# BrooksLabUCSC/splicedice

Measured on AMD Instinct MI355X. Metric: PS-matrix entries/sec (junctions x samples), higher is better.
Workload: dtype int32 counts -> f32 PS; 1 GPU; quant 2000000 junctions x 500 samples per GPU (north_star target size), cluster+PS; junctions_per_gpu=2000000, samples=500, counts=one seeded block of 200000 rows repeated down the matrix, parallelism=junction shards x1, one rank per GPU

## Files before the change

### splicedice_amd/csrc/cluster_fast.hip

```cpp
#include "common.h"

#ifndef SDICE_CLUSTER_ABLATE
#define SDICE_CLUSTER_ABLATE 0
#endif
#define SD_ABL(a, bit) (SDICE_CLUSTER_ABLATE && ((a).ablate & (bit)))

int sd_cluster_legacy(sdice_ctx* ctx, int64_t n, const int32_t* d_chrom, const int32_t* d_left, const int32_t* d_right,
                      const int8_t* d_strand, int32_t* d_row_of, int64_t* d_row_ptr, int64_t* nnz_out);

namespace {

constexpr int SPB = 8;
constexpr int BUCKET_MEAN = 2048;
constexpr int MAX_BUCKETS = 4096;
constexpr int SLOT_FACTOR = 8;
constexpr int64_t FAST_MAX_N = (int64_t)MAX_BUCKETS * BUCKET_MEAN;

enum : unsigned long long { ST_INVALID = 1, ST_SLOT_OVERFLOW = 2, ST_DUP = 4, ST_COL_OVERFLOW = 8, ST_LOOKBACK = 16 };
constexpr int SB_FLAGS = 0, SB_NNZ = 2, SB_MAXLEN = 32, SB_REACH = 64, SB_WORDS = 96;
constexpr int SB_STICKY = SB_WORDS, SB_ALLOC_WORDS = SB_WORDS + 8;
constexpr int SB_SLOTS = 32;

struct FastArgs {
    const int32_t* chrom; const int32_t* left; const int32_t* right; const int8_t* strand;
    int64_t n;
    int B;
    int S;
    int64_t slot_cap;
    int lds_cap;
    unsigned long long* sb;
    uint32_t* rank;
    uint32_t* col_done;
    uint64_t* spl;
    uint32_t* cursor;
    uint4* slots;
    uint32_t* rowC; uint32_t* rowL; uint32_t* rowR2;
    uint32_t* bmax64;
    unsigned long long* tile_state;
    int32_t* row_of; int64_t* row_ptr; int32_t* col; int64_t col_cap;
    uint32_t* blkneed;
    int spb;
    int sample_sort;
    int ablate;
};

__device__ __forceinline__ bool key_less(uint32_t ac, uint32_t al, uint32_t ar, uint32_t bc, uint32_t bl, uint32_t br) {
    return ac < bc || (ac == bc && (al < bl || (al == bl && ar < br)));
}
__device__ __forceinline__ bool elem_less(const uint4& a, const uint4& b) { return key_less(a.x, a.y, a.z, b.x, b.y, b.z); }

__device__ __forceinline__ int64_t sample_pos(int64_t i, int64_t n, int64_t S) {
    const int64_t stride = n / S;
    const uint64_t h = ((uint64_t)i * 0x9E3779B97F4A7C15ull) >> 33;
    return i * stride + (int64_t)(h % (uint64_t)stride);
}

__device__ __forceinline__ uint64_t sample_key(const FastArgs& a, int64_t i) {
    const int64_t p = sample_pos(i, a.n, a.S);
    return ((uint64_t)(uint32_t)a.chrom[p] << 32) | (uint64_t)(uint32_t)a.left[p];
}

__device__ __forceinline__ void count_less96(unsigned& c, uint64_t ka, uint32_t ia, uint64_t kb, uint32_t ib) {
    unsigned t;
    asm("v_sub_co_u32 %0, vcc, %2, %3\n\t"
        "v_subb_co_u32 %0, vcc, %4, %5, vcc\n\t"
        "v_subb_co_u32 %0, vcc, %6, %7, vcc\n\t"
        "v_addc_co_u32 %1, vcc, 0, %1, vcc"
        : "=&v"(t), "+v"(c)
        : "v"(ia), "v"(ib), "v"((unsigned)ka), "v"((unsigned)kb), "v"((unsigned)(ka >> 32)), "v"((unsigned)(kb >> 32))
        : "vcc");
}

__global__ void __launch_bounds__(256) sample_rank_kernel(FastArgs a) {
    __shared__ __align__(16) uint64_t jk[256];
    __shared__ unsigned last;
    const int t = threadIdx.x;
    if (blockIdx.x == 0 && blockIdx.y == 0 && t < SB_WORDS) a.sb[t] = 0ull;
    const int64_t i = (int64_t)blockIdx.x * 256 + t, j = (int64_t)blockIdx.y * 256 + t;
    jk[t] = j < a.S ? sample_key(a, j) : ~0ull;
    const uint64_t ik = i < a.S ? sample_key(a, i) : 0ull;
    __syncthreads();
    const int64_t j0 = (int64_t)blockIdx.y * 256;
    const int64_t split64 = i - j0;
    const uint32_t split = split64 < 0 ? 0u : split64 > 256 ? 256u : (uint32_t)split64;
    uint32_t cnt = 0;
#pragma unroll 8
    for (int q = 0; q < (SD_ABL(a, 8) ? 0 : 256); q += 2) {
        const ulonglong2 k2 = *reinterpret_cast<const ulonglong2*>(&jk[q]);
        count_less96(cnt, k2.x, (uint32_t)q, ik, split);
        count_less96(cnt, k2.y, (uint32_t)q + 1u, ik, split);
    }
    if (i < a.S && cnt) atomicAdd(&a.rank[i], cnt);
    asm volatile("s_waitcnt vmcnt(0)" ::: "memory");
    __syncthreads();
    if (t == 0) last = atomicAdd(&a.col_done[blockIdx.x], 1u) == gridDim.y - 1 ? 1u : 0u;
    __syncthreads();
    if (last && i < a.S) {
        const uint32_t rk = atomicAdd(&a.rank[i], 0u);
        if (rk != 0 && rk % (uint32_t)a.spb == 0) a.spl[rk / (uint32_t)a.spb - 1] = ik;
    }
}

constexpr int SC_KPT = 4;
template <int T>
__global__ void __launch_bounds__(T) bucket_scatter_kernel(FastArgs a) {
    extern __shared__ uint64_t sm64[];
    const int B = a.B;
    uint64_t* spl = sm64;
    uint32_t* cnt = reinterpret_cast<uint32_t*>(sm64 + B);
    uint32_t* base = cnt + B;
    __shared__ uint32_t wmax[T / 64];
    __shared__ uint32_t s_bad, s_over;
    const int t = threadIdx.x;
    if (t == 0) { s_bad = 0; s_over = 0; }
    for (int b = t; b < B; b += T) { spl[b] = b < B - 1 ? a.spl[b] : ~0ull; cnt[b] = 0; }
    __syncthreads();
    const int64_t tile0 = (int64_t)blockIdx.x * T * SC_KPT;
    uint32_t kc[SC_KPT], kl[SC_KPT], kr[SC_KPT], bk[SC_KPT], lr[SC_KPT];
    uint32_t maxlen = 0, bad = 0;
#pragma unroll
    for (int q = 0; q < SC_KPT; ++q) {
        const int64_t i = tile0 + q * T + t;
        bk[q] = 0xffffffffu;
        kc[q] = kl[q] = kr[q] = lr[q] = 0;
        if (i < a.n) {
            const int32_t c = a.chrom[i], l = a.left[i], r = a.right[i];
            const int st = a.strand[i];
            if (l < 0 || r < l || c < 0 || (st != 0 && st != 1)) bad = 1;
            else maxlen = max(maxlen, (uint32_t)(r - l));
            kc[q] = (uint32_t)c; kl[q] = (uint32_t)l; kr[q] = ((uint32_t)r << 1) | (uint32_t)(st & 1);
        }
    }
#pragma unroll
    for (int q = 0; q < SC_KPT; ++q) {
        if (tile0 + q * T + t < a.n) {
            const uint64_t k = ((uint64_t)kc[q] << 32) | kl[q];
            int lo = 0, hi = B - 1;
            while (lo < hi) {
                const int mid = (lo + hi) >> 1;
                if (spl[mid] <= k) lo = mid + 1; else hi = mid;
            }
            bk[q] = (uint32_t)lo;
            lr[q] = atomicAdd(&cnt[lo], 1u);
        }
    }
#pragma unroll
    for (int o = 32; o > 0; o >>= 1) maxlen = max(maxlen, (uint32_t)__shfl_xor((int)maxlen, o));
    if ((t & 63) == 0) wmax[t >> 6] = maxlen;
    if (bad) s_bad = 1;
    __syncthreads();
    for (int b = t; b < B; b += T) {
        const uint32_t c = cnt[b];
        base[b] = (c && !SD_ABL(a, 32)) ? atomicAdd(&a.cursor[b], c) : 0u;
    }
    if (t == 0) {
        uint32_t m = 0;
        for (int w = 0; w < T / 64; ++w) m = max(m, wmax[w]);
        if (m) atomicMax(&a.sb[SB_MAXLEN + (blockIdx.x % SB_SLOTS)], (unsigned long long)m);
    }
    __syncthreads();
#pragma unroll
    for (int q = 0; q < SC_KPT; ++q) {
        if (bk[q] == 0xffffffffu) continue;
        const int64_t i = tile0 + q * T + t;
        const uint64_t pos = (uint64_t)base[bk[q]] + lr[q];
        if (SD_ABL(a, 16)) continue;
        if (pos < (uint64_t)a.slot_cap) a.slots[(int64_t)bk[q] * a.slot_cap + (int64_t)pos] = make_uint4(kc[q], kl[q], kr[q], (uint32_t)i);
        else s_over = 1;
    }
    __syncthreads();
    if (t == 0 && (s_bad | s_over)) {
        const unsigned long long f = (s_bad ? (unsigned long long)ST_INVALID : 0ull) | (s_over ? (unsigned long long)ST_SLOT_OVERFLOW : 0ull);
        atomicOr(&a.sb[SB_FLAGS], f);
        atomicOr(&a.sb[SB_STICKY], f);
    }
}

__device__ __forceinline__ void cmpswap(uint4* buf, int lo, int hi) {
    const uint4 x = buf[lo], y = buf[hi];
    if (elem_less(y, x)) { buf[lo] = y; buf[hi] = x; }
}
__device__ __forceinline__ void cmpswap(uint64_t* buf, int lo, int hi) {
    const uint64_t x = buf[lo], y = buf[hi];
    buf[lo] = y < x ? y : x;
    buf[hi] = y < x ? x : y;
}

template <bool WAVE_LOCAL_OK, typename E>
__device__ __forceinline__ void bitonic_sort(E* buf, int count, int P, int t, int T) {
    const int half = P >> 1;
    bool prev_confined = false;
    for (int k = 2; k <= P; k <<= 1) {
        {
            const bool confined = WAVE_LOCAL_OK && k <= 128;
            if (confined && prev_confined) __builtin_amdgcn_wave_barrier(); else __syncthreads();
            prev_confined = confined;
            const int hk = k >> 1, lg = __ffs(hk) - 1;
            for (int c = t; c < half; c += T) {
// ... 362 lines not shown

__device__ __forceinline__ unsigned long long lookback_exclusive(unsigned long long* state, int tile, unsigned long long agg,
                                                                 int lane, unsigned long long* sb, bool fail) {
    if (lane == 0) st_agent(&state[tile], (tile == 0 ? LB_P : LB_A) | agg);
    unsigned long long excl = 0;
    int idx = tile - 1;
    unsigned spins = fail && tile == 1 ? (1u << 21) : 0u;
    while (idx >= 0) {
        const int j = idx - lane;
        const unsigned long long v = j >= 0 ? ld_agent(&state[j]) : LB_P;
        const unsigned flag = (unsigned)(v >> 62);
        const unsigned long long empty = __ballot(flag == 0u);
        const unsigned long long pm = __ballot(flag == 2u);
        const int first_p = pm ? __ffsll((long long)pm) - 1 : 64;
        const unsigned long long need = first_p >= 63 ? ~0ull : ((1ull << (first_p + 1)) - 1ull);
        if ((empty & need) || (fail && tile == 1)) {
            if (++spins > (1u << 21)) {
                if (lane == 0) { atomicOr(&sb[SB_FLAGS], (unsigned long long)ST_LOOKBACK); atomicOr(&sb[SB_STICKY], (unsigned long long)ST_LOOKBACK); }
                break;
            }
            __builtin_amdgcn_s_sleep(2);
            continue;
        }
        unsigned long long x = lane <= first_p ? (v & LB_MASK) : 0ull;
#pragma unroll
        for (int o = 32; o > 0; o >>= 1) x += __shfl_xor(x, o);
        excl += x;
        if (first_p < 64) break;
        idx -= 64;
    }
    if (lane == 0 && tile != 0) st_agent(&state[tile], LB_P | (excl + agg));
    return excl;
}

template <int T>
struct NbCfg {
    static constexpr int HB = 256;
    static constexpr int HF = 128;
    static constexpr int W = T + HB + HF;
    static constexpr int STAGE = 11 * T;
    static constexpr int KMAX = 16;
    static constexpr int WIN_WORDS = 6 * W;
    static constexpr int UNION_WORDS = WIN_WORDS > STAGE ? WIN_WORDS : STAGE;
};

template <class Emit>
__device__ __forceinline__ void walk_back_global(const FastArgs& a, int q, uint32_t c, uint32_t l, uint32_t st, uint32_t maxlen,
                                                 Emit emit) {
    while (q >= 0) {
        const uint32_t qc = a.rowC[q], ql = a.rowL[q], qr = a.rowR2[q];
        if (qc != c || ql + maxlen < l) break;
        if ((q & 63) == 63 && a.bmax64[q >> 6] < l) { q -= 64; continue; }
        if ((qr & 1u) == st && (qr >> 1) >= l) emit(q);
        --q;
    }
}
template <class Emit>
__device__ __forceinline__ void walk_fwd_global(const FastArgs& a, int q, int n, uint32_t c, uint32_t rgt, uint32_t st, Emit emit) {
    while (q < n) {
        const uint32_t qc = a.rowC[q], ql = a.rowL[q], qr = a.rowR2[q];
        if (qc != c || ql > rgt) break;
        if ((qr & 1u) == st) emit(q);
        ++q;
    }
}

template <int T>
__global__ void __launch_bounds__(T, 8) neighbours_kernel(FastArgs a) {
    typedef NbCfg<T> Cfg;
    constexpr int W = Cfg::W, KMAX = Cfg::KMAX;
    constexpr int EPT = (W + T - 1) / T;
    __shared__ __align__(16) uint32_t u_mem[Cfg::UNION_WORDS];
    __shared__ int16_t tmp[(KMAX + 1) * T];
    __shared__ uint32_t wsum[T / 64];
    __shared__ unsigned long long wmax0[T / 64], wmax1[T / 64];
    __shared__ uint32_t s_misc[4];
    __shared__ unsigned long long s_base;
    unsigned long long* cL = reinterpret_cast<unsigned long long*>(u_mem);
    unsigned long long* pm = cL + W;
    uint32_t* wR = reinterpret_cast<uint32_t*>(pm + W);
    uint16_t* rid = reinterpret_cast<uint16_t*>(wR + W);
    uint16_t* pos = rid + W;
    int32_t* stage = reinterpret_cast<int32_t*>(u_mem);
    const int t = threadIdx.x, lane = t & 63, w = __builtin_amdgcn_readfirstlane(t >> 6);
    const int n = (int)a.n;
    const int n_tiles = (n + T - 1) / T;
    const bool failed_chain = (a.sb[SB_FLAGS] & (ST_INVALID | ST_SLOT_OVERFLOW | ST_DUP)) != 0;
    __shared__ int s_tile;
    unsigned long long* ticket = a.tile_state + n_tiles;
    if (t == 0) s_tile = failed_chain ? (int)blockIdx.x : (int)atomicAdd(ticket, 1ull);
    __syncthreads();
#pragma nounroll
    for (int tile = s_tile; tile < n_tiles;) {
    const int t0 = tile * T;
    const int nr = min(T, n - t0);
    if (failed_chain) {
        if (t < nr) { a.row_ptr[t0 + t] = 0; if ((t & 15) == 0) a.blkneed[(t0 + t) >> 4] = 0; }
        if (t0 + t == 0) a.row_ptr[n] = 0;
        tile += gridDim.x;
        continue;
    }
    if (t == 0) s_misc[2] = 0;
    if (t < 64) {
        unsigned long long m = t < SB_SLOTS ? a.sb[SB_MAXLEN + t] : 0ull;
#pragma unroll
        for (int o = 32; o > 0; o >>= 1) { const unsigned long long y = __shfl_xor(m, o); m = y > m ? y : m; }
        if (t == 0) s_misc[1] = (uint32_t)m;
    }
    const int wlo = max(0, t0 - Cfg::HB), whi = min(n, t0 + nr + Cfg::HF);
    const int wn = whi - wlo;
    const uint32_t c0w = a.rowC[wlo];
    const uint32_t l0w = a.rowL[wlo];
    const int64_t cap = a.col_cap;
    int n1 = 0;
    {
        unsigned long long comp[EPT], own_cl[EPT], r0 = 0, r1 = 0;
        uint32_t rr[EPT], str[EPT], c1 = 0;
        unsigned long long v0[EPT], v1[EPT];
        uint32_t cb[EPT];
#pragma unroll
        for (int e = 0; e < EPT; ++e) {
            const int i = t * EPT + e;
            comp[e] = 0; own_cl[e] = 0; rr[e] = 0; str[e] = 0;
            cb[e] = c1;
            if (i < wn) {
                const uint32_t rc = a.rowC[wlo + i] - c0w, r2 = a.rowR2[wlo + i];
                own_cl[e] = ((unsigned long long)rc << 32) | a.rowL[wlo + i];
                rr[e] = r2 >> 1; str[e] = r2 & 1u;
                comp[e] = ((unsigned long long)rc << 32) | rr[e];
                if (str[e]) { r1 = comp[e] > r1 ? comp[e] : r1; ++c1; } else { r0 = comp[e] > r0 ? comp[e] : r0; }
            }
            v0[e] = r0; v1[e] = r1;
        }
        unsigned long long x0 = r0, x1 = r1;
        uint32_t xc = c1;
#pragma unroll
        for (int o = 1; o < 64; o <<= 1) {
            const unsigned long long y0 = __shfl_up(x0, o), y1 = __shfl_up(x1, o);
            const uint32_t yc = __shfl_up(xc, o);
            if (lane >= o) { x0 = y0 > x0 ? y0 : x0; x1 = y1 > x1 ? y1 : x1; xc += yc; }
        }
        if (lane == 63) { wmax0[w] = x0; wmax1[w] = x1; wsum[w] = xc; }
        __syncthreads();
        unsigned long long p0 = __shfl_up(x0, 1), p1 = __shfl_up(x1, 1);
        uint32_t pc = xc - c1;
        if (lane == 0) { p0 = 0; p1 = 0; }
#pragma unroll
        for (int k = 0; k < T / 64; ++k) {
            if (k < w) { p0 = wmax0[k] > p0 ? wmax0[k] : p0; p1 = wmax1[k] > p1 ? wmax1[k] : p1; pc += wsum[k]; }
            n1 += (int)wsum[k];
        }
#pragma unroll
        for (int e = 0; e < EPT; ++e) {
            const int i = t * EPT + e;
            if (i < wn) {
                const int before1 = (int)(pc + cb[e]);
                const int k = str[e] ? W - 1 - before1 : i - before1;
                const unsigned long long m = str[e] ? (v1[e] > p1 ? v1[e] : p1) : (v0[e] > p0 ? v0[e] : p0);
                cL[k] = own_cl[e]; pm[k] = m; wR[k] = rr[e]; rid[k] = (uint16_t)i; pos[i] = (uint16_t)k;
            }
        }
    }
    __syncthreads();
    const uint32_t maxlen = s_misc[1];
    const int n0 = wn - n1;

    const int r = t0 + t;
    const int ri = r - wlo;
    const bool act = t < nr;
    int p = 0;
    unsigned long long own = 0;
    uint32_t rgt = 0;
    if (act) { p = pos[ri]; own = cL[p]; rgt = wR[p]; }
    const uint32_t st = p >= W - n1 ? 1u : 0u;
    const uint32_t l = (uint32_t)own, crel = (uint32_t)(own >> 32), c = crel + c0w;
    const unsigned long long tb = own;
    const unsigned long long tf = (own & 0xffffffff00000000ull) | rgt;
    const bool exact = wlo == 0 || crel != 0 || l0w + maxlen < l;
    const int dfw = st ? -1 : 1;
    const int first = st ? W - 1 : 0;
    const int last = st ? W - n1 : n0 - 1;

    uint32_t deg = 0;
    int far_b = r, far_f = r;
    bool redo = false;
    auto emit_far = [&](int q) {
        const int d = q - r;
        if (deg < (uint32_t)KMAX) {
            if (d >= -32768 && d <= 32767) tmp[deg * T + t] = (int16_t)d; else redo = true;
        }
        ++deg;
        if (d < 0) far_b = q; else far_f = q;
    };
    if (act && !SD_ABL(a, 64)) {
        int16_t* mytmp = tmp + t;
        auto take = [&](bool hit, int wi) {
            const uint32_t slot = (hit & (deg < (uint32_t)KMAX)) ? deg : (uint32_t)KMAX;
            mytmp[slot * T] = (int16_t)(wi - ri);
            deg += hit ? 1u : 0u;
            return hit ? wlo + wi : -1;
        };
        const int up = (p - first) * dfw, ulast = (last - first) * dfw;
        if (exact) {
            int u = up - 1;
            for (;;) {
                const int q0 = first + dfw * max(u, 0), q1 = first + dfw * max(u - 1, 0);
                const unsigned long long m0 = pm[q0], m1 = pm[q1];
                const uint32_t x0 = wR[q0], x1 = wR[q1];
                const int i0 = rid[q0], i1 = rid[q1];
                if (!((u >= 0) & (m0 >= tb))) break;
                const int f0 = take(x0 >= l, i0);
                far_b = f0 >= 0 ? f0 : far_b;
                --u;
                if (!((u >= 0) & (m1 >= tb))) break;
                const int f1 = take(x1 >= l, i1);
                far_b = f1 >= 0 ? f1 : far_b;
                --u;
            }
            if (u < 0 && wlo > 0) walk_back_global(a, wlo - 1, c, l, st, maxlen, emit_far);
        } else {
            walk_back_global(a, r - 1, c, l, st, maxlen, emit_far);
        }
        {
            int u = up + 1;
            for (;;) {
                const int q0 = first + dfw * min(u, ulast), q1 = first + dfw * min(u + 1, ulast);
                const unsigned long long c0 = cL[q0], c1 = cL[q1];
                const int i0 = rid[q0], i1 = rid[q1];
                if (!((u <= ulast) & (c0 <= tf))) break;
                far_f = take(true, i0);
                ++u;
                if (!((u <= ulast) & (c1 <= tf))) break;
                far_f = take(true, i1);
                ++u;
            }
            if (u > ulast && whi < n) walk_fwd_global(a, whi, n, c, rgt, st, emit_far);
        }
        if (deg > (uint32_t)KMAX) redo = true;
    }
    uint32_t reach = (uint32_t)max(r - far_b, far_f - r);
    {
        const int b16 = t & 15;
        const unsigned lo_n = act ? (unsigned)min(max(r - far_b - b16, 0), 255) : 0u;
        const unsigned hi_n = act ? (unsigned)min(max(far_f - r - (15 - b16), 0), 255) : 0u;
        typedef unsigned short us2 __attribute__((ext_vector_type(2)));
        us2 pk = {(unsigned short)lo_n, (unsigned short)hi_n};
#pragma unroll
        for (int o = 8; o > 0; o >>= 1) {
            const unsigned y = (unsigned)__shfl_xor((int)__builtin_bit_cast(unsigned, pk), o);
            pk = __builtin_elementwise_max(pk, __builtin_bit_cast(us2, y));
        }
        if (act && b16 == 0) a.blkneed[r >> 4] = (uint32_t)pk.x | ((uint32_t)pk.y << 8);
    }
    uint32_t x = deg;
#pragma unroll
    for (int o = 1; o < 64; o <<= 1) { const uint32_t y = __shfl_up(x, o); if (lane >= o) x += y; }
#pragma unroll
    for (int o = 32; o > 0; o >>= 1) reach = max(reach, (uint32_t)__shfl_xor((int)reach, o));
    if (lane == 63) wsum[w] = x;
    if (lane == 0 && reach) atomicMax(&s_misc[2], reach);
    __syncthreads();
    uint32_t wbase = 0, total = 0;
#pragma unroll
    for (int k = 0; k < T / 64; ++k) { const uint32_t v = wsum[k]; if (k < w) wbase += v; total += v; }
    const uint32_t loff = wbase + x - deg;
    if (w == 0) {
        const unsigned long long base = SD_ABL(a, 128) ? 0ull : lookback_exclusive(a.tile_state, tile, (unsigned long long)total, lane, a.sb, (a.ablate & 256) != 0);
        if (lane == 0) {
            s_base = base;
            if (s_misc[2]) atomicMax(&a.sb[SB_REACH + (tile % SB_SLOTS)], (unsigned long long)s_misc[2]);
        }
    }
    const bool staged = total <= (uint32_t)Cfg::STAGE;
    if (staged && act && deg) {
        if (!redo) {
            for (uint32_t k = 0; k < deg; ++k) stage[loff + k] = r + (int)tmp[k * T + t];
        } else {
            uint32_t k = loff;
            walk_back_global(a, r - 1, c, l, st, maxlen, [&](int q) { stage[k++] = q; });
            walk_fwd_global(a, r + 1, n, c, rgt, st, [&](int q) { stage[k++] = q; });
        }
    }
    __syncthreads();
    const int64_t base = (int64_t)s_base;
    if (act) a.row_ptr[r] = min(base + (int64_t)loff, cap);
    if (tile == n_tiles - 1 && t == 0) {
        a.row_ptr[n] = min(base + (int64_t)total, cap);
        a.sb[SB_NNZ] = (unsigned long long)(base + (int64_t)total);
        if (base + (int64_t)total > cap) { atomicOr(&a.sb[SB_FLAGS], (unsigned long long)ST_COL_OVERFLOW); atomicOr(&a.sb[SB_STICKY], (unsigned long long)ST_COL_OVERFLOW); }
    }
    if (staged) {
        for (uint32_t k = t; k < total; k += T)
            if (base + k < cap) a.col[base + k] = stage[k];
    } else if (act && deg) {
        int64_t k = base + loff;
        auto put = [&](int q) { if (k < cap) a.col[k] = q; ++k; };
        walk_back_global(a, r - 1, c, l, st, maxlen, put);
        walk_fwd_global(a, r + 1, n, c, rgt, st, put);
    }
    if (t == 0) s_tile = (int)atomicAdd(ticket, 1ull);
    __syncthreads();
    tile = s_tile;
    }
}

inline unsigned grid_for(int64_t n, int threads) { return (unsigned)sd_ceil_div(n, threads); }

struct FastPlan {
    FastArgs a;
    size_t zero_bytes;
    void* zero_base;
    size_t k4_zero_bytes;
    int n_tiles;
};

constexpr int NB_T = 512;

int fast_plan(sdice_ctx* ctx, int64_t n, const int32_t* d_chrom, const int32_t* d_left, const int32_t* d_right,
              const int8_t* d_strand, int32_t* d_row_of, int64_t* d_row_ptr, FastPlan& pl) {
    FastArgs& a = pl.a;
    a.chrom = d_chrom; a.left = d_left; a.right = d_right; a.strand = d_strand; a.n = n;
    static_assert(kSdParams[SD_P_CLUSTER_BUCKET_MEAN].dflt == BUCKET_MEAN, "the default is the largest mean the kernels take");
    int64_t bucket_mean = ctx->param(SD_P_CLUSTER_BUCKET_MEAN);
    if (bucket_mean < 256 || bucket_mean > BUCKET_MEAN) bucket_mean = BUCKET_MEAN;
    int64_t B = sd_ceil_div(n, bucket_mean);
    if (B < 1) B = 1;
    if (B > MAX_BUCKETS) B = MAX_BUCKETS;
    a.B = (int)B;
    a.spb = (int)ctx->param(SD_P_CLUSTER_SPB);
    if (a.spb < 2 || a.spb > 64) a.spb = n <= ((int64_t)2 << 20) ? 12 : SPB;
    a.S = B > 1 ? (int)(B * a.spb) : 0;
    const int64_t mean = sd_ceil_div(n, B);
    a.slot_cap = B > 1 ? (mean * SLOT_FACTOR < n ? mean * SLOT_FACTOR : n) : n;
    int64_t lds_cap = ctx->param(SD_P_CLUSTER_LDS_CAP);
    if (lds_cap <= 0 || lds_cap > 8192) lds_cap = 8192;
    if (lds_cap < 2) lds_cap = 2;
    a.lds_cap = (int)lds_cap;
    a.sample_sort = ctx->param(SD_P_CLUSTER_SAMPLE_SORT) != 0;
    pl.n_tiles = (int)sd_ceil_div(n, NB_T);
    const size_t nb64 = (size_t)sd_ceil_div(n, 64) + 2;
    if (!ctx->cluster_sb) {
        hipError_t e = hipMalloc((void**)&ctx->cluster_sb, (size_t)SB_ALLOC_WORDS * 8);
        if (e != hipSuccess) {
            sdice_set_error("sdice_cluster: hipMalloc of the status block failed: %s", hipGetErrorString(e));
            return SDICE_ERR_NOMEM;
        }
        SD_HIP(hipMemsetAsync(ctx->cluster_sb, 0, (size_t)SB_ALLOC_WORDS * 8, ctx->stream));
    }
    const size_t zk4 = ((size_t)pl.n_tiles + 2) * 8;
    const size_t n_cd = (size_t)(a.S + 255) / 256 + 4;
    const size_t zrest = (size_t)a.B * 4 + (size_t)(a.S + 4) * 4 + nb64 * 4 + n_cd * 4;
    const size_t slots_bytes = (size_t)a.B * (size_t)a.slot_cap * 16;
    const size_t total = zk4 + zrest + slots_bytes + (size_t)n * 12 + (size_t)a.B * 16 + 16 * 4096;
    SD_TRY(ctx->arena.reserve(total, ctx->stream));
    Arena& A = ctx->arena;
    char* z = (char*)A.alloc(zk4 + zrest + 1024);
    a.slots = (uint4*)A.alloc(slots_bytes);
    a.rowC = (uint32_t*)A.alloc((size_t)n * 4);
    a.rowL = (uint32_t*)A.alloc((size_t)n * 4);
    a.rowR2 = (uint32_t*)A.alloc((size_t)n * 4);
    a.spl = (uint64_t*)A.alloc((size_t)a.B * 8 + 8);
    if (!z || !a.slots || !a.rowC || !a.rowL || !a.rowR2 || !a.spl) return SDICE_ERR_NOMEM;
    pl.zero_base = z;
    pl.k4_zero_bytes = zk4;
    pl.zero_bytes = zk4 + zrest;
    a.sb = (unsigned long long*)ctx->cluster_sb;
    a.tile_state = (unsigned long long*)z;
    a.cursor = (uint32_t*)(z + zk4);
    a.rank = a.cursor + a.B;
    a.bmax64 = a.rank + a.S + 4;
    a.col_done = a.bmax64 + nb64;
    a.row_of = d_row_of; a.row_ptr = d_row_ptr;
    a.ablate = (int)ctx->param(SD_P_CLUSTER_ABLATE);
    return SDICE_OK;
}

int launch_neighbours(sdice_ctx* ctx, FastPlan& pl) {
    pl.a.col = ctx->d_col;
    pl.a.col_cap = ctx->col_cap;
    pl.a.blkneed = ctx->d_reach;
    static int per_cu = 0;
    if (per_cu == 0) {
        int occ = 0;
        SD_HIP(hipOccupancyMaxActiveBlocksPerMultiprocessor(&occ, reinterpret_cast<const void*>(neighbours_kernel<NB_T>), NB_T, 0));
        per_cu = occ > 0 ? occ : 1;
    }
    int64_t grid = std::min<int64_t>(pl.n_tiles, (int64_t)per_cu * ctx->n_cu);
    const int64_t forced = ctx->param(SD_P_CLUSTER_NB_GRID);
    if (forced > 0) grid = std::min<int64_t>(grid, forced);
    SD_LAUNCH(ctx, "neighbours_kernel", (neighbours_kernel<NB_T>), dim3((unsigned)std::max<int64_t>(grid, 1)), dim3(NB_T), 0, pl.a);
    return SDICE_OK;
}

int ensure_col(sdice_ctx* ctx, int64_t want) {
    if (want <= ctx->col_cap) return SDICE_OK;
    if (ctx->d_col) {
        SD_HIP(hipStreamSynchronize(ctx->stream));
        (void)hipFree(ctx->d_col);
    }
    ctx->d_col = nullptr;
    ctx->col_cap = 0;
    hipError_t e = hipMalloc((void**)&ctx->d_col, (size_t)want * 4);
    if (e != hipSuccess) {
        sdice_set_error("sdice_cluster: hipMalloc of %lld neighbour indices failed: %s", (long long)want, hipGetErrorString(e));
        return SDICE_ERR_NOMEM;
    }
    ctx->col_cap = want;
    return SDICE_OK;
}

int ensure_reach(sdice_ctx* ctx, int64_t n) {
    n = sd_ceil_div(n, 16) + 1;
    if (n <= ctx->reach_cap) return SDICE_OK;
    if (ctx->d_reach) {
        SD_HIP(hipStreamSynchronize(ctx->stream));
        (void)hipFree(ctx->d_reach);
    }
    ctx->d_reach = nullptr;
    ctx->reach_cap = 0;
    hipError_t e = hipMalloc((void**)&ctx->d_reach, (size_t)n * 4);
    if (e != hipSuccess) {
        sdice_set_error("sdice_cluster: hipMalloc of %lld block-reach entries failed: %s", (long long)n, hipGetErrorString(e));
        return SDICE_ERR_NOMEM;
    }
    ctx->reach_cap = n;
    return SDICE_OK;
}

}

static int fast_fetch_status(sdice_ctx* ctx, unsigned long long* flags, int64_t* nnz, int64_t* reach, unsigned long long* sticky = nullptr) {
    int64_t* hp = ctx->h_pinned;
    SD_HIP(hipMemcpyAsync(hp, ctx->cluster_sb, (size_t)SB_ALLOC_WORDS * 8, hipMemcpyDeviceToHost, ctx->stream));
    SD_HIP(hipMemsetAsync((unsigned long long*)ctx->cluster_sb + SB_STICKY, 0, 8, ctx->stream));
    SD_HIP(hipStreamSynchronize(ctx->stream));
    if (sticky) *sticky = (unsigned long long)hp[SB_STICKY];
    *flags = (unsigned long long)hp[SB_FLAGS];
    *nnz = hp[SB_NNZ];
    int64_t rc = 0;
    for (int i = 0; i < SB_SLOTS; ++i) rc = hp[SB_REACH + i] > rc ? hp[SB_REACH + i] : rc;
    *reach = rc;
    return SDICE_OK;
}

static int fast_flags_to_error(unsigned long long flags) {
    if (flags & ST_INVALID) {
        sdice_set_error("sdice_cluster: invalid junction (need 0 <= left <= right, chrom_rank >= 0, strand in {0,1})");
        return SDICE_ERR_ARG;
    }
    if (flags & ST_DUP) {
        sdice_set_error("sdice_cluster: duplicate junction (chrom, left, right, strand): the junctions must be distinct");
        return SDICE_ERR_ARG;
    }
    return SDICE_OK;
}

int sd_cluster_resolve(sdice_ctx* ctx) {
    if (!ctx->cluster_pending) return SDICE_OK;
    ctx->cluster_pending = false;
    unsigned long long flags = 0, sticky = 0;
    int64_t nnz = 0, reach = 0;
    SD_TRY(fast_fetch_status(ctx, &flags, &nnz, &reach, &sticky));
    ctx->nnz = 0;
    flags |= sticky;
    SD_TRY(fast_flags_to_error(flags));
    if (flags & (ST_SLOT_OVERFLOW | ST_LOOKBACK)) {
        sdice_set_error("sdice_cluster_dev (asynchronous): %s; call with nnz != NULL (synchronous) "
                        "to take the generic path", (flags & ST_LOOKBACK) ? "the look-back gave up waiting" : "a sort bucket overflowed");
        return SDICE_ERR_STATE;
    }
    if (flags & ST_COL_OVERFLOW) {
        sdice_set_error("sdice_cluster_dev (asynchronous): %lld neighbour entries exceed the list capacity %lld; "
                        "call once with nnz != NULL (synchronous) to size it", (long long)nnz, (long long)ctx->col_cap);
        return SDICE_ERR_STATE;
    }
    ctx->nnz = nnz;
    ctx->cluster_reach = (int)reach;
    return SDICE_OK;
}

extern "C" int sdice_cluster_status(sdice_ctx* ctx, int64_t* nnz, int32_t* reach) {
    SD_ARG(ctx, "ctx is NULL");
    SD_TRY(sd_cluster_resolve(ctx));
    if (nnz) *nnz = ctx->nnz;
    if (reach) *reach = ctx->cluster_reach;
    return SDICE_OK;
}

extern "C" int sdice_cluster_dev(sdice_ctx* ctx, int64_t n, const int32_t* d_chrom, const int32_t* d_left,
                                 const int32_t* d_right, const int8_t* d_strand, int32_t* d_row_of,
                                 int64_t* d_row_ptr, int64_t* nnz_out) {
    SD_ARG(ctx, "ctx is NULL");
    SD_ARG(n >= 0 && n < ((int64_t)1 << 31), "n out of range");
    SD_HIP(hipSetDevice(ctx->device));
    if (nnz_out && ctx->cluster_pending) SD_TRY(sd_cluster_resolve(ctx));
    ctx->reach_n = 0;
    const bool legacy = n > FAST_MAX_N || ctx->param(SD_P_CLUSTER_GENERIC) || ctx->param(SD_P_CLUSTER_LEGACY);
    if ((legacy || n == 0) && ctx->cluster_pending) SD_TRY(sd_cluster_resolve(ctx));
    if (legacy || n == 0) return sd_cluster_legacy(ctx, n, d_chrom, d_left, d_right, d_strand, d_row_of, d_row_ptr, nnz_out);
    SD_ARG(d_chrom && d_left && d_right && d_strand && d_row_of && d_row_ptr, "NULL pointer");
    ctx->nnz = 0;
    ctx->cluster_reach = 0;
    if (nnz_out) *nnz_out = 0;

    FastPlan pl;
    SD_TRY(fast_plan(ctx, n, d_chrom, d_left, d_right, d_strand, d_row_of, d_row_ptr, pl));
    FastArgs& a = pl.a;
    SD_TRY(ensure_col(ctx, 16 * n + 1024));
    SD_TRY(ensure_reach(ctx, n));

    SD_HIP(hipMemsetAsync(pl.zero_base, 0, pl.zero_bytes, ctx->stream));
    if (a.S == 0) SD_HIP(hipMemsetAsync(a.sb, 0, (size_t)SB_WORDS * 8, ctx->stream));
    if (a.S > 0) {
        const unsigned g = grid_for(a.S, 256);
        SD_LAUNCH(ctx, "sample_rank_kernel", sample_rank_kernel, dim3(g, g), dim3(256), 0, a);
    }
    {
        const size_t lds = (size_t)a.B * 16;
        if (n <= (1 << 19)) {
            SD_HIP(hipFuncSetAttribute(reinterpret_cast<const void*>(bucket_scatter_kernel<512>),
                                       hipFuncAttributeMaxDynamicSharedMemorySize, (int)lds));
            SD_LAUNCH(ctx, "bucket_scatter_kernel", (bucket_scatter_kernel<512>), dim3(grid_for(n, 512 * SC_KPT)), dim3(512), lds, a);
        } else {
            SD_HIP(hipFuncSetAttribute(reinterpret_cast<const void*>(bucket_scatter_kernel<1024>),
                                       hipFuncAttributeMaxDynamicSharedMemorySize, (int)lds));
            SD_LAUNCH(ctx, "bucket_scatter_kernel", (bucket_scatter_kernel<1024>), dim3(grid_for(n, 1024 * SC_KPT)), dim3(1024), lds, a);
        }
    }
    {
        const size_t lds = SORT_LDS_BYTES;
        SD_HIP(hipFuncSetAttribute(reinterpret_cast<const void*>(bucket_sort_kernel),
                                   hipFuncAttributeMaxDynamicSharedMemorySize, (int)lds));
        SD_LAUNCH(ctx, "bucket_sort_kernel", bucket_sort_kernel, dim3((unsigned)a.B), dim3(SORT_T), lds, a);
    }
    SD_TRY(launch_neighbours(ctx, pl));

    if (!nnz_out) {
        ctx->cluster_pending = true;
        ctx->reach_n = n;
        return SDICE_OK;
    }
    unsigned long long flags = 0;
    int64_t nnz = 0, reach = 0;
    SD_TRY(fast_fetch_status(ctx, &flags, &nnz, &reach));
    SD_TRY(fast_flags_to_error(flags));
    if (flags & (ST_SLOT_OVERFLOW | ST_LOOKBACK))
        return sd_cluster_legacy(ctx, n, d_chrom, d_left, d_right, d_strand, d_row_of, d_row_ptr, nnz_out);
    if (flags & ST_COL_OVERFLOW) {
        SD_TRY(sd_cluster_check_nnz(ctx, nnz, false));
        SD_TRY(ensure_col(ctx, nnz + nnz / 8 + 1024));
        SD_HIP(hipMemsetAsync(pl.zero_base, 0, pl.k4_zero_bytes, ctx->stream));
        SD_HIP(hipMemsetAsync(a.sb, 0, (size_t)SB_MAXLEN * 8, ctx->stream));
        SD_HIP(hipMemsetAsync(a.sb + SB_REACH, 0, (size_t)SB_SLOTS * 8, ctx->stream));
        SD_TRY(launch_neighbours(ctx, pl));
        SD_TRY(fast_fetch_status(ctx, &flags, &nnz, &reach));
        if (flags) {
            sdice_set_error("sdice_cluster: neighbour pass failed after resizing (flags %llu)", flags);
            return SDICE_ERR_STATE;
        }
    }
    ctx->nnz = nnz;
    ctx->cluster_reach = (int)reach;
    ctx->reach_n = n;
    *nnz_out = nnz;
    return SDICE_OK;
}
```

### splicedice_amd/csrc/common.h

```cpp
#pragma once
#include <hip/hip_runtime.h>
#include <stdint.h>
#include <map>
#include <string>
#include <vector>
#include "sdice.h"
#include "params.h"

void sdice_set_error(const char* fmt, ...);

#define SD_HIP(expr)                                                                   \
    do {                                                                               \
        hipError_t _e = (expr);                                                        \
        if (_e != hipSuccess) {                                                        \
            sdice_set_error("%s:%d: %s -> %s", __FILE__, __LINE__, #expr,              \
                            hipGetErrorString(_e));                                    \
            return SDICE_ERR_HIP;                                                      \
        }                                                                              \
    } while (0)

#define SD_TRY(expr)                                                                   \
    do {                                                                               \
        int _s = (expr);                                                               \
        if (_s != SDICE_OK) return _s;                                                 \
    } while (0)

#define SD_ARG(cond, msg)                                                              \
    do {                                                                               \
        if (!(cond)) {                                                                 \
            sdice_set_error("%s: %s", __func__, msg);                                  \
            return SDICE_ERR_ARG;                                                      \
        }                                                                              \
    } while (0)

struct ProfPending {
    int name_id;
    hipEvent_t e0, e1;
};

struct ProfStat {
    int64_t launches = 0;
    double total_ms = 0.0;
};

struct Arena {
    struct Chunk { char* p; size_t cap; size_t off; };
    std::vector<Chunk> chunks;
    void* alloc(size_t bytes);
    int reset(hipStream_t s);
    int reserve(size_t total, hipStream_t s);
    void release();
};

struct sdice_ctx {
    int device = 0;
    hipStream_t stream = nullptr;
    int n_cu = 0;
    int64_t hbm_bytes = 0;
    char dev_name[128] = {0};

    Arena arena;

    int32_t* d_col = nullptr;
    int64_t col_cap = 0;
    int64_t nnz = 0;
    int cluster_reach = 0;
    uint32_t* d_reach = nullptr;
    int64_t reach_cap = 0;
    int64_t reach_n = 0;
    int64_t* h_pinned = nullptr;
    void* cluster_sb = nullptr;
    bool cluster_pending = false;

    double* d_lf = nullptr;
    int64_t lf_n = 0;
    uint64_t fisher_steps[2] = {0, 0};

    bool prof_on = false;
    int prof_mode = 0;
    std::vector<std::string> prof_names;
    std::map<std::string, int> prof_ids;
    std::vector<ProfStat> prof_stats;
    std::vector<ProfPending> prof_pending;
    std::vector<hipEvent_t> event_pool;
    hipEvent_t t0 = nullptr, t1 = nullptr;

    int64_t params[SD_P_COUNT];
    sdice_ctx() {
        for (int i = 0; i < SD_P_COUNT; ++i) params[i] = kSdParams[i].dflt;
    }

    void* rccl_lib = nullptr;
    void* comm = nullptr;
    int rank = 0, world = 1;
    hipStream_t comm_stream = nullptr;
    hipEvent_t comm_ev = nullptr;
    bool comm_forked = false;
    hipStream_t coll_stream() const { return comm_forked ? comm_stream : stream; }

    int64_t param(SdParam which) const { return params[which]; }
};

int sd_prof_begin(sdice_ctx* ctx, const char* name);
void sd_prof_end(sdice_ctx* ctx, int token);
int sd_prof_drain(sdice_ctx* ctx);

#define SD_LAUNCH(ctx, name, kernel, grid, block, shmem, ...)                          \
    do {                                                                               \
        int _tok = sd_prof_begin((ctx), (name));                                       \
        hipLaunchKernelGGL(kernel, (grid), (block), (shmem), (ctx)->stream, __VA_ARGS__); \
        sd_prof_end((ctx), _tok);                                                      \
        SD_HIP(hipGetLastError());                                                     \
    } while (0)

static inline int64_t sd_ceil_div(int64_t a, int64_t b) { return (a + b - 1) / b; }

class HostStaging {
  public:
    explicit HostStaging(sdice_ctx* ctx) : ctx_(ctx) {}
    ~HostStaging();
    HostStaging(const HostStaging&) = delete;
    HostStaging& operator=(const HostStaging&) = delete;

    template <class T> int alloc(T** d, int64_t count) {
        void* p = nullptr;
        const int rc = sdice_dmalloc(ctx_, count * (int64_t)sizeof(T), &p);
        if (p) bufs_.push_back(p);
        *d = static_cast<T*>(p);
        return rc;
    }
    template <class T> int upload(T** d, const T* h, int64_t count) {
        SD_TRY(alloc(d, count));
        return sdice_h2d(ctx_, *d, h, count * (int64_t)sizeof(T));
    }
    template <class T> int download(T* h, const T* d, int64_t count) {
        return sdice_d2h(ctx_, h, d, count * (int64_t)sizeof(T));
    }

  private:
    sdice_ctx* ctx_;
    std::vector<void*> bufs_;
};

int sd_check_csr(const char* who, int64_t n_out, int64_t n_rows, const int64_t* row_ptr, const int32_t* col);

constexpr int64_t SD_MAX_PAIRS = (int64_t)8192 * 8191 / 2;
int sd_check_pair_list(const char* who, int32_t s, int64_t m, const int32_t* pairs);

int sd_cluster_resolve(sdice_ctx* ctx);
int sd_cluster_check_nnz(sdice_ctx* ctx, int64_t nnz, bool host);

int sd_radix_sort_pairs(sdice_ctx* ctx, int64_t n, const uint64_t* d_keys_in, const uint32_t* d_vals_in,
                        uint64_t* d_keys_out, uint32_t* d_vals_out, uint64_t* d_keys_tmp, uint32_t* d_vals_tmp,
                        uint64_t bit_mask);
int sd_radix_sort_pairs_segmented(sdice_ctx* ctx, int64_t n, int64_t segs, const uint64_t* d_keys_in,
// ... 4 lines not shown
```

### splicedice_amd/csrc/ctx.hip

```cpp
#include "common.h"
#include <stdarg.h>
#include <stdio.h>
#include <string.h>

static thread_local char g_err[1024] = "";

void sdice_set_error(const char* fmt, ...) {
    va_list ap;
    va_start(ap, fmt);
    vsnprintf(g_err, sizeof(g_err), fmt, ap);
    va_end(ap);
}

extern "C" const char* sdice_last_error(void) { return g_err; }
extern "C" int sdice_version(void) { return SDICE_ABI_VERSION; }

void* Arena::alloc(size_t bytes) {
    bytes = (bytes + 255) & ~size_t(255);
    if (bytes == 0) bytes = 256;
    if (!chunks.empty()) {
        Chunk& c = chunks.back();
        if (c.off + bytes <= c.cap) {
            void* p = c.p + c.off;
            c.off += bytes;
// ... 24 lines not shown
        for (auto& c : chunks) { total += c.cap; (void)hipFree(c.p); }
        chunks.clear();
        char* p = nullptr;
        if (hipMalloc((void**)&p, total) == hipSuccess) chunks.push_back({p, total, 0});
    } else if (chunks.size() == 1) {
        chunks[0].off = 0;
    }
    return SDICE_OK;
}

int Arena::reserve(size_t total, hipStream_t s) {
    total = (total + 4095) & ~size_t(4095);
    if (chunks.size() == 1 && chunks[0].cap >= total) {
        chunks[0].off = 0;
        return SDICE_OK;
    }
    if (!chunks.empty()) {
        SD_HIP(hipStreamSynchronize(s));
        release();
    }
    char* p = nullptr;
    hipError_t e = hipMalloc((void**)&p, total);
    if (e != hipSuccess) {
        sdice_set_error("arena: hipMalloc(%zu) failed: %s", total, hipGetErrorString(e));
        return SDICE_ERR_NOMEM;
    }
    chunks.push_back({p, total, 0});
    return SDICE_OK;
}

void Arena::release() {
    for (auto& c : chunks) (void)hipFree(c.p);
    chunks.clear();
}

extern "C" int sdice_ctx_create(int device_ordinal, sdice_ctx** out) {
    SD_ARG(out != nullptr, "out is NULL");
    *out = nullptr;
    int count = 0;
    hipError_t e = hipGetDeviceCount(&count);
    if (e != hipSuccess || count <= 0) {
        sdice_set_error("sdice_ctx_create: no HIP device available (%s); there is no CPU backend",
                        e != hipSuccess ? hipGetErrorString(e) : "device count 0");
        return SDICE_ERR_HIP;
    }
    SD_ARG(device_ordinal >= 0 && device_ordinal < count, "device ordinal out of range");
    SD_HIP(hipSetDevice(device_ordinal));
    hipDeviceProp_t prop;
    SD_HIP(hipGetDeviceProperties(&prop, device_ordinal));
    if (strncmp(prop.gcnArchName, "gfx950", 6) != 0) {
        sdice_set_error("sdice_ctx_create: device %d is %s; this library ships gfx950 (MI355X) code only",
                        device_ordinal, prop.gcnArchName);
        return SDICE_ERR_HIP;
    }
    sdice_ctx* ctx = new sdice_ctx();
    ctx->device = device_ordinal;
    ctx->n_cu = prop.multiProcessorCount;
    ctx->hbm_bytes = (int64_t)prop.totalGlobalMem;
    snprintf(ctx->dev_name, sizeof(ctx->dev_name), "%s (%s)", prop.name, prop.gcnArchName);
    if (hipStreamCreateWithFlags(&ctx->stream, hipStreamNonBlocking) != hipSuccess ||
        hipEventCreate(&ctx->t0) != hipSuccess || hipEventCreate(&ctx->t1) != hipSuccess ||
        hipHostMalloc((void**)&ctx->h_pinned, 16384) != hipSuccess) {
        sdice_set_error("sdice_ctx_create: stream/event/pinned allocation failed");
        delete ctx;
        return SDICE_ERR_HIP;
    }
    *out = ctx;
    return SDICE_OK;
}

extern "C" int sdice_ctx_destroy(sdice_ctx* ctx) {
    if (!ctx) return SDICE_OK;
    (void)hipSetDevice(ctx->device);
    (void)hipStreamSynchronize(ctx->stream);
    sdice_comm_destroy(ctx);
    for (auto& p : ctx->prof_pending) { ctx->event_pool.push_back(p.e0); ctx->event_pool.push_back(p.e1); }
    for (auto ev : ctx->event_pool) (void)hipEventDestroy(ev);
    if (ctx->t0) (void)hipEventDestroy(ctx->t0);
    if (ctx->t1) (void)hipEventDestroy(ctx->t1);
    if (ctx->d_col) (void)hipFree(ctx->d_col);
    if (ctx->d_reach) (void)hipFree(ctx->d_reach);
    if (ctx->d_lf) (void)hipFree(ctx->d_lf);
    if (ctx->cluster_sb) (void)hipFree(ctx->cluster_sb);
    if (ctx->h_pinned) (void)hipHostFree(ctx->h_pinned);
    ctx->arena.release();
    if (ctx->comm_stream) { (void)hipStreamSynchronize(ctx->comm_stream); (void)hipStreamDestroy(ctx->comm_stream); }
    if (ctx->comm_ev) (void)hipEventDestroy(ctx->comm_ev);
    (void)hipStreamDestroy(ctx->stream);
    delete ctx;
    return SDICE_OK;
}

extern "C" int sdice_sync(sdice_ctx* ctx) {
    SD_ARG(ctx, "ctx is NULL");
    if (ctx->comm_forked) SD_TRY(sdice_comm_join(ctx));
    SD_HIP(hipStreamSynchronize(ctx->stream));
    return sd_cluster_resolve(ctx);
}

extern "C" int sdice_trim(sdice_ctx* ctx) {
    SD_ARG(ctx, "ctx is NULL");
    SD_HIP(hipSetDevice(ctx->device));
    SD_HIP(hipStreamSynchronize(ctx->stream));
    ctx->arena.release();
    return sd_cluster_resolve(ctx);
}

extern "C" int sdice_device_info(sdice_ctx* ctx, char* name, int name_cap, int* compute_units,
                                 int64_t* hbm_bytes) {
    SD_ARG(ctx, "ctx is NULL");
    if (name && name_cap > 0) snprintf(name, name_cap, "%s", ctx->dev_name);
    if (compute_units) *compute_units = ctx->n_cu;
    if (hbm_bytes) *hbm_bytes = ctx->hbm_bytes;
    return SDICE_OK;
}

extern "C" int sdice_dmalloc(sdice_ctx* ctx, int64_t bytes, void** dptr) {
    SD_ARG(ctx && dptr && bytes >= 0, "bad arguments");
    *dptr = nullptr;
    SD_HIP(hipSetDevice(ctx->device));
    hipError_t e = hipMalloc(dptr, bytes > 0 ? (size_t)bytes : 256);
    if (e != hipSuccess) {
        sdice_set_error("sdice_dmalloc(%lld): %s", (long long)bytes, hipGetErrorString(e));
        return SDICE_ERR_NOMEM;
    }
    return SDICE_OK;
}

extern "C" int sdice_dfree(sdice_ctx* ctx, void* dptr) {
    SD_ARG(ctx, "ctx is NULL");
    if (!dptr) return SDICE_OK;
    SD_HIP(hipStreamSynchronize(ctx->stream));
    SD_HIP(hipFree(dptr));
    return SDICE_OK;
}

extern "C" int sdice_h2d(sdice_ctx* ctx, void* dst_dev, const void* src_host, int64_t bytes) {
    SD_ARG(ctx && bytes >= 0, "bad arguments");
    if (bytes == 0) return SDICE_OK;
    SD_ARG(dst_dev && src_host, "NULL pointer");
    SD_HIP(hipMemcpyAsync(dst_dev, src_host, (size_t)bytes, hipMemcpyHostToDevice, ctx->stream));
    SD_HIP(hipStreamSynchronize(ctx->stream));
    return SDICE_OK;
}

extern "C" int sdice_d2h(sdice_ctx* ctx, void* dst_host, const void* src_dev, int64_t bytes) {
    SD_ARG(ctx && bytes >= 0, "bad arguments");
    if (bytes == 0) return SDICE_OK;
    SD_ARG(dst_host && src_dev, "NULL pointer");
    SD_HIP(hipMemcpyAsync(dst_host, src_dev, (size_t)bytes, hipMemcpyDeviceToHost, ctx->stream));
    SD_HIP(hipStreamSynchronize(ctx->stream));
    return SDICE_OK;
}

HostStaging::~HostStaging() {
    if (bufs_.empty()) return;
    (void)hipStreamSynchronize(ctx_->stream);
    for (void* p : bufs_) (void)hipFree(p);
}

extern "C" int sdice_dmemset(sdice_ctx* ctx, void* dptr, int value, int64_t bytes) {
    SD_ARG(ctx && bytes >= 0, "bad arguments");
    if (bytes == 0) return SDICE_OK;
    SD_HIP(hipMemsetAsync(dptr, value, (size_t)bytes, ctx->stream));
    return SDICE_OK;
}
// ... 152 lines not shown
```

Measured before the change: 535.8 billion entries/s.

## Fold cluster scratch zeroing into kernels and hoist neighbour maxlen reduction

Removes the upfront hipMemsetAsync of the cluster scratch region. That zeroing now happens inside sample_rank_kernel, and the rank/col_done array moves to a persistent context buffer that bucket_scatter_kernel re-zeroes after use, so no memset is needed on the next call. In neighbours_kernel, the maxlen reduction is hoisted out of the per-tile loop and kept in registers, and the row loads are issued up front to overlap their latency. The cost is extra grid-stride stores inside the kernels and dirty-flag state that has to be tracked correctly across calls and errors.

```diff
diff --git a/splicedice_amd/csrc/cluster_fast.hip b/splicedice_amd/csrc/cluster_fast.hip
--- a/splicedice_amd/csrc/cluster_fast.hip
+++ b/splicedice_amd/csrc/cluster_fast.hip
@@ -31,6 +31,9 @@
     unsigned long long* sb;
     uint32_t* rank;
     uint32_t* col_done;
+    int64_t rank_words;
+    uint32_t* zero32;
+    int64_t zero32_n;
     uint64_t* spl;
     uint32_t* cursor;
     uint4* slots;
@@ -76,6 +79,10 @@
     __shared__ unsigned last;
     const int t = threadIdx.x;
     if (blockIdx.x == 0 && blockIdx.y == 0 && t < SB_WORDS) a.sb[t] = 0ull;
+    {
+        const int64_t threads = (int64_t)gridDim.x * gridDim.y * 256;
+        for (int64_t k = ((int64_t)blockIdx.y * gridDim.x + blockIdx.x) * 256 + t; k < a.zero32_n; k += threads) a.zero32[k] = 0u;
+    }
     const int64_t i = (int64_t)blockIdx.x * 256 + t, j = (int64_t)blockIdx.y * 256 + t;
     jk[t] = j < a.S ? sample_key(a, j) : ~0ull;
     const uint64_t ik = i < a.S ? sample_key(a, i) : 0ull;
@@ -114,6 +121,7 @@
     const int t = threadIdx.x;
     if (t == 0) { s_bad = 0; s_over = 0; }
     for (int b = t; b < B; b += T) { spl[b] = b < B - 1 ? a.spl[b] : ~0ull; cnt[b] = 0; }
+    for (int64_t k = (int64_t)blockIdx.x * T + t; k < a.rank_words; k += (int64_t)gridDim.x * T) a.rank[k] = 0u;
     __syncthreads();
     const int64_t tile0 = (int64_t)blockIdx.x * T * SC_KPT;
     uint32_t kc[SC_KPT], kl[SC_KPT], kr[SC_KPT], bk[SC_KPT], lr[SC_KPT];
@@ -642,16 +650,26 @@
     uint16_t* rid = reinterpret_cast<uint16_t*>(wR + W);
     uint16_t* pos = rid + W;
     int32_t* stage = reinterpret_cast<int32_t*>(u_mem);
-    const int t = threadIdx.x, lane = t & 63, w = __builtin_amdgcn_readfirstlane(t >> 6);
     const int n = (int)a.n;
     const int n_tiles = (n + T - 1) / T;
     const bool failed_chain = (a.sb[SB_FLAGS] & (ST_INVALID | ST_SLOT_OVERFLOW | ST_DUP)) != 0;
+    uint32_t maxlen;
+    {
+        const int l0 = (int)(threadIdx.x & 63u);
+        unsigned long long m = l0 < SB_SLOTS ? a.sb[SB_MAXLEN + l0] : 0ull;
+#pragma unroll
+        for (int o = 32; o > 0; o >>= 1) { const unsigned long long y = __shfl_xor(m, o); m = y > m ? y : m; }
+        maxlen = (uint32_t)__builtin_amdgcn_readfirstlane((int)(uint32_t)m);
+    }
     __shared__ int s_tile;
     unsigned long long* ticket = a.tile_state + n_tiles;
-    if (t == 0) s_tile = failed_chain ? (int)blockIdx.x : (int)atomicAdd(ticket, 1ull);
+    if (threadIdx.x == 0) s_tile = failed_chain ? (int)blockIdx.x : (int)atomicAdd(ticket, 1ull);
     __syncthreads();
 #pragma nounroll
     for (int tile = s_tile; tile < n_tiles;) {
+    int t = threadIdx.x;
+    asm volatile("" : "+v"(t));
+    const int lane = t & 63, w = __builtin_amdgcn_readfirstlane(t >> 6);
     const int t0 = tile * T;
     const int nr = min(T, n - t0);
     if (failed_chain) {
@@ -661,12 +679,6 @@
         continue;
     }
     if (t == 0) s_misc[2] = 0;
-    if (t < 64) {
-        unsigned long long m = t < SB_SLOTS ? a.sb[SB_MAXLEN + t] : 0ull;
-#pragma unroll
-        for (int o = 32; o > 0; o >>= 1) { const unsigned long long y = __shfl_xor(m, o); m = y > m ? y : m; }
-        if (t == 0) s_misc[1] = (uint32_t)m;
-    }
     const int wlo = max(0, t0 - Cfg::HB), whi = min(n, t0 + nr + Cfg::HF);
     const int wn = whi - wlo;
     const uint32_t c0w = a.rowC[wlo];
@@ -678,14 +690,20 @@
         uint32_t rr[EPT], str[EPT], c1 = 0;
         unsigned long long v0[EPT], v1[EPT];
         uint32_t cb[EPT];
+        uint32_t ldc[EPT], ldl[EPT], ldr[EPT];
+#pragma unroll
+        for (int e = 0; e < EPT; ++e) {
+            const int i = wlo + min(t * EPT + e, wn - 1);
+            ldc[e] = a.rowC[i]; ldl[e] = a.rowL[i]; ldr[e] = a.rowR2[i];
+        }
 #pragma unroll
         for (int e = 0; e < EPT; ++e) {
             const int i = t * EPT + e;
             comp[e] = 0; own_cl[e] = 0; rr[e] = 0; str[e] = 0;
             cb[e] = c1;
             if (i < wn) {
-                const uint32_t rc = a.rowC[wlo + i] - c0w, r2 = a.rowR2[wlo + i];
-                own_cl[e] = ((unsigned long long)rc << 32) | a.rowL[wlo + i];
+                const uint32_t rc = ldc[e] - c0w, r2 = ldr[e];
+                own_cl[e] = ((unsigned long long)rc << 32) | ldl[e];
                 rr[e] = r2 >> 1; str[e] = r2 & 1u;
                 comp[e] = ((unsigned long long)rc << 32) | rr[e];
                 if (str[e]) { r1 = comp[e] > r1 ? comp[e] : r1; ++c1; } else { r0 = comp[e] > r0 ? comp[e] : r0; }
@@ -722,7 +740,6 @@
         }
     }
     __syncthreads();
-    const uint32_t maxlen = s_misc[1];
     const int n0 = wn - n1;
 
     const int r = t0 + t;
@@ -821,10 +838,12 @@
     if (lane == 0 && reach) atomicMax(&s_misc[2], reach);
     __syncthreads();
     uint32_t wbase = 0, total = 0;
-#pragma unroll
-    for (int k = 0; k < T / 64; ++k) { const uint32_t v = wsum[k]; if (k < w) wbase += v; total += v; }
+    int ws = w;
+    asm volatile("" : "+s"(ws));
+#pragma unroll
+    for (int k = 0; k < T / 64; ++k) { const uint32_t v = wsum[k]; if (k < ws) wbase += v; total += v; }
     const uint32_t loff = wbase + x - deg;
-    if (w == 0) {
+    if (ws == 0) {
         const unsigned long long base = SD_ABL(a, 128) ? 0ull : lookback_exclusive(a.tile_state, tile, (unsigned long long)total, lane, a.sb, (a.ablate & 256) != 0);
         if (lane == 0) {
             s_base = base;
@@ -907,9 +926,26 @@
         }
         SD_HIP(hipMemsetAsync(ctx->cluster_sb, 0, (size_t)SB_ALLOC_WORDS * 8, ctx->stream));
     }
+    const size_t n_cd = (size_t)(a.S + 255) / 256 + 4;
+    a.rank_words = a.S > 0 ? (int64_t)(a.S + 4 + n_cd) : 0;
+    if (a.rank_words > ctx->cluster_rank_words) {
+        if (ctx->cluster_rank) {
+            SD_HIP(hipStreamSynchronize(ctx->stream));
+            (void)hipFree(ctx->cluster_rank);
+        }
+        ctx->cluster_rank = nullptr;
+        ctx->cluster_rank_words = 0;
+        const int64_t want = std::max<int64_t>(a.rank_words, 1 << 16);
+        hipError_t e = hipMalloc((void**)&ctx->cluster_rank, (size_t)want * 4);
+        if (e != hipSuccess) {
+            sdice_set_error("sdice_cluster: hipMalloc of the sample ranks failed: %s", hipGetErrorString(e));
+            return SDICE_ERR_NOMEM;
+        }
+        ctx->cluster_rank_words = want;
+        ctx->cluster_rank_dirty = true;
+    }
     const size_t zk4 = ((size_t)pl.n_tiles + 2) * 8;
-    const size_t n_cd = (size_t)(a.S + 255) / 256 + 4;
-    const size_t zrest = (size_t)a.B * 4 + (size_t)(a.S + 4) * 4 + nb64 * 4 + n_cd * 4;
+    const size_t zrest = (size_t)a.B * 4 + nb64 * 4;
     const size_t slots_bytes = (size_t)a.B * (size_t)a.slot_cap * 16;
     const size_t total = zk4 + zrest + slots_bytes + (size_t)n * 12 + (size_t)a.B * 16 + 16 * 4096;
     SD_TRY(ctx->arena.reserve(total, ctx->stream));
@@ -927,9 +963,11 @@
     a.sb = (unsigned long long*)ctx->cluster_sb;
     a.tile_state = (unsigned long long*)z;
     a.cursor = (uint32_t*)(z + zk4);
-    a.rank = a.cursor + a.B;
-    a.bmax64 = a.rank + a.S + 4;
-    a.col_done = a.bmax64 + nb64;
+    a.bmax64 = a.cursor + a.B;
+    a.rank = ctx->cluster_rank;
+    a.col_done = a.rank + a.S + 4;
+    a.zero32 = (uint32_t*)z;
+    a.zero32_n = a.S > 0 ? (int64_t)((zk4 + zrest) / 4) : 0;
     a.row_of = d_row_of; a.row_ptr = d_row_ptr;
     a.ablate = (int)ctx->param(SD_P_CLUSTER_ABLATE);
     return SDICE_OK;
@@ -1069,9 +1107,12 @@
     SD_TRY(ensure_col(ctx, 16 * n + 1024));
     SD_TRY(ensure_reach(ctx, n));
 
-    SD_HIP(hipMemsetAsync(pl.zero_base, 0, pl.zero_bytes, ctx->stream));
-    if (a.S == 0) SD_HIP(hipMemsetAsync(a.sb, 0, (size_t)SB_WORDS * 8, ctx->stream));
-    if (a.S > 0) {
+    if (a.S == 0) {
+        SD_HIP(hipMemsetAsync(pl.zero_base, 0, pl.zero_bytes, ctx->stream));
+        SD_HIP(hipMemsetAsync(a.sb, 0, (size_t)SB_WORDS * 8, ctx->stream));
+    } else {
+        if (ctx->cluster_rank_dirty) SD_HIP(hipMemsetAsync(ctx->cluster_rank, 0, (size_t)ctx->cluster_rank_words * 4, ctx->stream));
+        ctx->cluster_rank_dirty = true;
         const unsigned g = grid_for(a.S, 256);
         SD_LAUNCH(ctx, "sample_rank_kernel", sample_rank_kernel, dim3(g, g), dim3(256), 0, a);
     }
@@ -1086,6 +1127,7 @@
                                        hipFuncAttributeMaxDynamicSharedMemorySize, (int)lds));
             SD_LAUNCH(ctx, "bucket_scatter_kernel", (bucket_scatter_kernel<1024>), dim3(grid_for(n, 1024 * SC_KPT)), dim3(1024), lds, a);
         }
+        if (a.S > 0) ctx->cluster_rank_dirty = false;
     }
     {
         const size_t lds = SORT_LDS_BYTES;
diff --git a/splicedice_amd/csrc/common.h b/splicedice_amd/csrc/common.h
--- a/splicedice_amd/csrc/common.h
+++ b/splicedice_amd/csrc/common.h
@@ -71,6 +71,9 @@
     int64_t* h_pinned = nullptr;
     void* cluster_sb = nullptr;
     bool cluster_pending = false;
+    uint32_t* cluster_rank = nullptr;
+    int64_t cluster_rank_words = 0;
+    bool cluster_rank_dirty = false;
 
     double* d_lf = nullptr;
     int64_t lf_n = 0;
diff --git a/splicedice_amd/csrc/ctx.hip b/splicedice_amd/csrc/ctx.hip
--- a/splicedice_amd/csrc/ctx.hip
+++ b/splicedice_amd/csrc/ctx.hip
@@ -130,6 +130,7 @@
     if (ctx->d_reach) (void)hipFree(ctx->d_reach);
     if (ctx->d_lf) (void)hipFree(ctx->d_lf);
     if (ctx->cluster_sb) (void)hipFree(ctx->cluster_sb);
+    if (ctx->cluster_rank) (void)hipFree(ctx->cluster_rank);
     if (ctx->h_pinned) (void)hipHostFree(ctx->h_pinned);
     ctx->arena.release();
     if (ctx->comm_stream) { (void)hipStreamSynchronize(ctx->comm_stream); (void)hipStreamDestroy(ctx->comm_stream); }
```

Result: no change. 538.2 billion entries/s, median of 4 (+0.4%).
